# apache/arrow-rs

Measured on NVIDIA H100. Metric: Mrows/sec filter+take+add on 1e9-row Int64/Float64; % HBM roofline, higher is better.
Workload: dtype i64 (filter/take/sum) + f64 (add)

## Files before the change

arrow-rs_b200/csrc/bitmap.cu:

```cuda
#include "bitmap.cuh"

__global__ void __launch_bounds__(256) k_bitmap_and(const uint8_t *__restrict__ a, int64_t aoff,
                                                    const uint8_t *__restrict__ b, int64_t boff,
                                                    int64_t len, uint64_t *__restrict__ out,
                                                    unsigned long long *__restrict__ res) {
  int64_t words = (len + 63) >> 6;
  int64_t stride = (int64_t)gridDim.x * blockDim.x;
  unsigned cnt = 0;
  for (int64_t w = (int64_t)blockIdx.x * blockDim.x + threadIdx.x; w < words; w += stride) {
    uint64_t x = ld_bits64(a, aoff + (w << 6), aoff + len);
    if (b) x &= ld_bits64(b, boff + (w << 6), boff + len);
    if (out) out[w] = x;
    cnt += __popcll(x);
  }
  if (res) {
    cnt = warp_sum(cnt);
    if ((threadIdx.x & 31) == 0 && cnt) atomicAdd(res + RES_COUNT, (unsigned long long)cnt);
  }
}

acu_status acu_bitmap_and_launch(acu_ctx *ctx, const uint8_t *a, int64_t aoff, const uint8_t *b,
                                 int64_t boff, int64_t len, uint64_t *out, bool count, unsigned long long *res) {
  if (len <= 0) return ACU_OK;
  int64_t words = (len + 63) >> 6;
  ACU_LAUNCH(ctx, k_bitmap_and, acu_grid(ctx, (words + 255) / 256, 8), 256, 0, a, aoff, b, boff, len, out,
             count ? (res ? res : ctx->d_res) : nullptr);
  return ACU_OK;
}

int64_t acu_resolve_null_count(acu_ctx *ctx, const acu_array *a, acu_status *st) {
  *st = ACU_OK;
  if (!a->validity) return 0;
  if (a->null_count >= 0) return a->null_count;
  int64_t len = a->is_scalar ? 1 : a->len;
  if (len == 0) return 0;
  if (ctx->async_on) {
    *st = acu_fail(ctx, ACU_ERR_INVALID_ARGUMENT, -1, 0, 0, 0,
                   "null_count = -1 needs a device count (a synchronisation): pass the cached null_count inside an async section");
    return 0;
  }
  if ((*st = acu_res_reset(ctx)) != ACU_OK) return 0;
  if ((*st = acu_bitmap_and_launch(ctx, a->validity, a->validity_offset, nullptr, 0, len, nullptr, true)) != ACU_OK) return 0;
  if ((*st = acu_res_fetch(ctx)) != ACU_OK) return 0;
  return len - (int64_t)ctx->h_res[RES_COUNT];
}

extern "C" acu_status acu_bitmap_count(acu_ctx *ctx, const uint8_t *bits, int64_t offset,
                                       const uint8_t *validity, int64_t validity_offset, int64_t len,
                                       int64_t *out_count) {
  ACU_ENTER(ctx);
  *out_count = 0;
  if (len <= 0) return ACU_OK;
  ACU_TRY(acu_res_reset(ctx));
  ACU_TRY(acu_bitmap_and_launch(ctx, bits, offset, validity, validity_offset, len, nullptr, true));
  ACU_TRY(acu_res_fetch(ctx));
  *out_count = (int64_t)ctx->h_res[RES_COUNT];
  return ACU_OK;
}
```

arrow-rs_b200/csrc/elementwise.cu:

```cuda
#include <stdio.h>

#include <algorithm>
#include <limits>
#include <type_traits>

#include "bitmap.cuh"
#include "internal.cuh"

namespace {

template <class T, int EPL> struct alignas(EPL * sizeof(T) == 16 ? 16 : sizeof(T)) Pack { T v[EPL]; };

template <class T, int EPL>
__device__ __forceinline__ Pack<T, EPL> pack_load(const T *p) {
  Pack<T, EPL> r;
  if constexpr (EPL * sizeof(T) == 16) {
    uint4 x = ld_stream16(p);
    r = *reinterpret_cast<Pack<T, EPL> *>(&x);
  } else {
    static_assert(EPL == 1, "scalar path");
    r.v[0] = __ldg(p);
  }
  return r;
}
template <class T, int EPL>
__device__ __forceinline__ void pack_store(T *p, Pack<T, EPL> r) {
  if constexpr (EPL * sizeof(T) == 16) {
    st_stream16(p, *reinterpret_cast<uint4 *>(&r));
  } else {
    *p = r.v[0];
  }
}

__device__ __forceinline__ uint64_t ones_to(int64_t row, int64_t n) {
  int64_t k = n - row;
  return k >= 64 ? ~0ull : (k <= 0 ? 0ull : ((~0ull) >> (64 - k)));
}

enum { CLS_WRAP = 0, CLS_CHECKED = 1, CLS_DIVREM = 2, CLS_DECIMAL = 3 };
enum { OP_ADD = 0, OP_SUB = 1, OP_MUL = 2, OP_DIV = 3, OP_REM = 4, OP_NEG = 5 };

template <class T> struct is_fp { static constexpr bool value = std::is_floating_point<T>::value; };

__device__ __forceinline__ double fp_add(double a, double b) { return __dadd_rn(a, b); }
__device__ __forceinline__ double fp_sub(double a, double b) { return __dsub_rn(a, b); }
__device__ __forceinline__ double fp_mul(double a, double b) { return __dmul_rn(a, b); }
__device__ __forceinline__ double fp_div(double a, double b) { return __ddiv_rn(a, b); }
__device__ __forceinline__ double fp_rem(double a, double b) { return fmod(a, b); }
__device__ __forceinline__ float fp_add(float a, float b) { return __fadd_rn(a, b); }
__device__ __forceinline__ float fp_sub(float a, float b) { return __fsub_rn(a, b); }
__device__ __forceinline__ float fp_mul(float a, float b) { return __fmul_rn(a, b); }
__device__ __forceinline__ float fp_div(float a, float b) { return __fdiv_rn(a, b); }
__device__ __forceinline__ float fp_rem(float a, float b) { return fmodf(a, b); }

template <class T, int CLS>
__device__ __forceinline__ bool apply_op(int op, T l, T r, T &o) {
  if constexpr (is_fp<T>::value) {
    if constexpr (CLS == CLS_DIVREM) {
      o = (op == OP_DIV) ? fp_div(l, r) : fp_rem(l, r);
    } else {
      o = (op == OP_ADD) ? fp_add(l, r) : (op == OP_SUB) ? fp_sub(l, r) : (op == OP_MUL) ? fp_mul(l, r) : -r;
    }
    return false;
  } else {
    using U = typename std::make_unsigned<T>::type;
    constexpr bool SIGNED = std::is_signed<T>::value;
    if constexpr (CLS == CLS_WRAP) {
      U a = (U)l, b = (U)r;
      o = (T)((op == OP_ADD) ? (U)(a + b) : (op == OP_SUB) ? (U)(a - b) : (op == OP_MUL) ? (U)(a * b) : (U)((U)0 - b));
      return false;
    } else if constexpr (CLS == CLS_CHECKED) {
      if constexpr (sizeof(T) < 8) {
        using W = typename std::conditional<SIGNED, int64_t, uint64_t>::type;
        W a = (W)l, b = (W)r;
        W w = (op == OP_ADD) ? a + b : (op == OP_SUB) ? a - b : (op == OP_MUL) ? a * b : (W)0 - b;
        o = (T)w;
        if constexpr (SIGNED) return w < (W)std::numeric_limits<T>::min() || w > (W)std::numeric_limits<T>::max();
        else return (op == OP_SUB) ? (a < b) : (op == OP_NEG ? false : w > (W)std::numeric_limits<T>::max());
      } else if constexpr (SIGNED) {
        int64_t a = l, b = r;
        if (op == OP_NEG) { a = 0; }
        if (op == OP_ADD) {
          int64_t s = (int64_t)((uint64_t)a + (uint64_t)b);
          o = s;
          return ((a ^ s) & (b ^ s)) < 0;
        } else if (op == OP_MUL) {
          int64_t lo = (int64_t)((uint64_t)a * (uint64_t)b);
          int64_t hi = __mul64hi(a, b);
          o = lo;
          return hi != (lo >> 63);
        } else {
          int64_t s = (int64_t)((uint64_t)a - (uint64_t)b);
          o = s;
          return ((a ^ b) & (a ^ s)) < 0;
        }
      } else {
        uint64_t a = l, b = r;
        if (op == OP_ADD) { o = a + b; return o < a; }
        if (op == OP_MUL) { o = a * b; return __umul64hi(a, b) != 0; }
        if (op == OP_NEG) { o = (uint64_t)0 - b; return false; }
        o = a - b;
        return a < b;
      }
    } else {
      o = 0;
      if (r == 0) return true;
      if constexpr (SIGNED) {
        if (r == (T)-1) {
          if (op == OP_DIV) {
            if (l == std::numeric_limits<T>::min()) return true;
            o = (T)(-l);
          }
          return false;
        }
      }
      o = (op == OP_DIV) ? (T)(l / r) : (T)(l % r);
      return false;
    }
  }
}

template <class T> struct dec_unsigned;
template <> struct dec_unsigned<int32_t> { using type = uint32_t; };
template <> struct dec_unsigned<int64_t> { using type = uint64_t; };
template <> struct dec_unsigned<__int128> { using type = unsigned __int128; };
template <class T> __host__ __device__ __forceinline__ T dec_min() {
  return (T)((typename dec_unsigned<T>::type)1 << (8 * sizeof(T) - 1));
}

__host__ __device__ __forceinline__ uint64_t umul64hi(uint64_t a, uint64_t b) {
#ifdef __CUDA_ARCH__
  return __umul64hi(a, b);
#else
  return (uint64_t)(((unsigned __int128)a * b) >> 64);
#endif
}
__host__ __device__ __forceinline__ int64_t mul64hi(int64_t a, int64_t b) {
#ifdef __CUDA_ARCH__
  return __mul64hi(a, b);
#else
  return (int64_t)(((__int128)a * b) >> 64);
#endif
}

template <class T> __host__ __device__ __forceinline__ bool add_ovf(T a, T b, T &o) {
  using U = typename dec_unsigned<T>::type;
  const T s = (T)((U)a + (U)b);
  o = s;
  return ((a ^ s) & (b ^ s)) < 0;
}
template <class T> __host__ __device__ __forceinline__ bool sub_ovf(T a, T b, T &o) {
  using U = typename dec_unsigned<T>::type;
  const T s = (T)((U)a - (U)b);
  o = s;
  return ((a ^ b) & (a ^ s)) < 0;
}
__host__ __device__ __forceinline__ bool mul_ovf(int32_t a, int32_t b, int32_t &o) {
  const int64_t w = (int64_t)a * b;
  o = (int32_t)w;
  return w != (int64_t)o;
}
__host__ __device__ __forceinline__ bool mul_ovf(int64_t a, int64_t b, int64_t &o) {
  const int64_t lo = (int64_t)((uint64_t)a * (uint64_t)b);
  o = lo;
  return mul64hi(a, b) != (lo >> 63);
}
__host__ __device__ __forceinline__ bool mul_ovf(__int128 a, __int128 b, __int128 &o) {
  const int64_t a64 = (int64_t)a, b64 = (int64_t)b;
  if ((__int128)a64 == a && (__int128)b64 == b) {
    const uint64_t lo = (uint64_t)a64 * (uint64_t)b64;
    o = (__int128)(((unsigned __int128)(uint64_t)mul64hi(a64, b64) << 64) | lo);
    return false;
  }
  using U = unsigned __int128;
  const bool neg = (a < 0) != (b < 0);
  const U ua = a < 0 ? (U)0 - (U)a : (U)a, ub = b < 0 ? (U)0 - (U)b : (U)b;
  const uint64_t ah = (uint64_t)(ua >> 64), al = (uint64_t)ua, bh = (uint64_t)(ub >> 64), bl = (uint64_t)ub;
  if (ah && bh) return true;
  const uint64_t x = ah ? ah : bh, y = ah ? bl : al;
  if (umul64hi(x, y)) return true;
  const uint64_t cross = x * y;
  const uint64_t hi = umul64hi(al, bl) + cross;
  if (hi < cross) return true;
  const U m = ((U)hi << 64) | (U)(al * bl);
  if (m > ((U)1 << 127) - (neg ? 0 : 1)) return true;
  o = neg ? (__int128)((U)0 - m) : (__int128)m;
  return false;
}
template <class T> __host__ __device__ __forceinline__ bool divrem_ovf(bool is_div, T l, T r, T &o) {
  o = T();
  if (r == T()) return true;
  if (r == (T)-1) {
    if (l == dec_min<T>()) return true;
    if (is_div) o = (T)(T() - l);
    return false;
  }
  if constexpr (sizeof(T) == 16) {
    const int64_t l64 = (int64_t)l, r64 = (int64_t)r;
    if ((__int128)l64 == l && (__int128)r64 == r) {
      o = is_div ? l64 / r64 : l64 % r64;
      return false;
    }
  }
  o = is_div ? (T)(l / r) : (T)(l % r);
  return false;
}
template <class T> __host__ __device__ __forceinline__ bool dec_apply(int op, T l, T r, T l_mul, T r_mul, T &o) {
  o = T();
  if (op == OP_NEG) return sub_ovf<T>(T(), r, o);
  if (op == OP_MUL) return mul_ovf(l, r, o);
  if (l_mul != (T)1 && mul_ovf(l, l_mul, l)) return true;
  if (r_mul != (T)1 && mul_ovf(r, r_mul, r)) return true;
  if (op == OP_ADD) return add_ovf<T>(l, r, o);
  if (op == OP_SUB) return sub_ovf<T>(l, r, o);
  return divrem_ovf<T>(op == OP_DIV, l, r, o);
}

template <class T>
struct ArithParams {
  const T *a, *b;
  T *out;
  int64_t n;
  const uint8_t *av, *bv;
  int64_t aoff, boff;
  uint64_t *out_valid;
  unsigned long long *res;
  int op;
  int a_scalar, b_scalar;
  int zero_nulls;
  T l_mul, r_mul;
};

template <class T, int CLS>
__device__ __forceinline__ bool row_op(const ArithParams<T> &p, T l, T r, T &o) {
  if constexpr (CLS == CLS_DECIMAL) return dec_apply<T>(p.op, l, r, p.l_mul, p.r_mul, o);
  else return apply_op<T, CLS>(p.op, l, r, o);
}

template <class T, int CLS, int EPL>
__global__ void __launch_bounds__(256, (CLS == CLS_WRAP ? 4 : (CLS == CLS_DECIMAL && sizeof(T) == 16) ? 2 : 3))
    k_arith(const ArithParams<T> p) {
  constexpr bool WIDE = CLS == CLS_DECIMAL && sizeof(T) == 16;
  constexpr int R = (32 * EPL > 64) ? 32 * EPL : 64;
  constexpr int LPS = R / (32 * EPL);
  constexpr int U = (LPS >= 2 && !WIDE) ? 2 : 4;
  constexpr int GROUP = U * R;
  constexpr int SG = 2048;
  constexpr int GPS = SG / GROUP;
  constexpr bool fallible = (CLS != CLS_WRAP) && !is_fp<T>::value;
  const int lane = threadIdx.x & 31;
  const int64_t warp = ((int64_t)blockIdx.x * blockDim.x + threadIdx.x) >> 5;
  const int64_t nwarps = ((int64_t)gridDim.x * blockDim.x) >> 5;
  const int64_t n = p.n;
  const int64_t sgroups = n / SG;
  const bool has_valid = p.out_valid != nullptr;
  T sa = T(), sb = T();
  if (p.a_scalar) sa = ldg_elem(p.a);
  if (p.b_scalar) sb = ldg_elem(p.b);
  unsigned valid_cnt = 0;
  unsigned long long err = ~0ull;

  for (int64_t sg = warp; sg < sgroups; sg += nwarps) {
    const int64_t sbase = sg * SG;
    uint64_t vw = ~0ull;
    if (has_valid) {
      const int64_t row = sbase + lane * 64;
      if (p.av) vw &= ld_bits64(p.av, p.aoff + row, p.aoff + n);
      if (p.bv) vw &= ld_bits64(p.bv, p.boff + row, p.boff + n);
      p.out_valid[row >> 6] = vw;
      valid_cnt += __popcll(vw);
    }
#pragma unroll 1
    for (int gi = 0; gi < GPS; ++gi) {
      const int64_t base = sbase + gi * GROUP;
      const T *__restrict__ pa = p.a + base + lane * EPL;
      const T *__restrict__ pb = p.b + base + lane * EPL;
      Pack<T, EPL> va[U * LPS], vb[U * LPS];
#pragma unroll
      for (int k = 0; k < U * LPS; ++k) {
        if (!p.a_scalar) va[k] = pack_load<T, EPL>(pa + k * 32 * EPL);
        if (!p.b_scalar) vb[k] = pack_load<T, EPL>(pb + k * 32 * EPL);
      }
      T *__restrict__ po = p.out + base + lane * EPL;
#pragma unroll
      for (int k = 0; k < U * LPS; ++k) {
        uint32_t bits = ~0u;
        if (fallible && p.zero_nulls) {
          const int pos = gi * GROUP + k * 32 * EPL + lane * EPL;
          const uint64_t w = __shfl_sync(ACU_FULL_MASK, vw, pos >> 6);
          bits = (uint32_t)(w >> (pos & 63));
        }
        Pack<T, EPL> o;
#pragma unroll
        for (int e = 0; e < EPL; ++e) {
          const T l = p.a_scalar ? sa : va[k].v[e];
          const T r = p.b_scalar ? sb : vb[k].v[e];
          T x;
          const bool bad = row_op<T, CLS>(p, l, r, x);
          if (fallible) {
            if (!((bits >> e) & 1u)) x = T();
            else if (bad) {
              const unsigned long long i = (unsigned long long)(base + k * 32 * EPL + lane * EPL + e);
              err = i < err ? i : err;
            }
          }
          o.v[e] = x;
        }
        pack_store<T, EPL>(po + k * 32 * EPL, o);
      }
    }
  }

  if (warp == 0) {
    for (int64_t row = sgroups * SG; row < n; row += 64) {
      uint64_t vw = ones_to(row, n);
      if (has_valid) {
        if (p.av) vw &= ld_bits64(p.av, p.aoff + row, p.aoff + n);
        if (p.bv) vw &= ld_bits64(p.bv, p.boff + row, p.boff + n);
        if (lane == 0) { p.out_valid[row >> 6] = vw; valid_cnt += __popcll(vw); }
      }
#pragma unroll
      for (int h = 0; h < 2; ++h) {
        const int64_t i = row + h * 32 + lane;
        if (i >= n) continue;
        const T l = p.a_scalar ? sa : ldg_elem(p.a + i);
        const T r = p.b_scalar ? sb : ldg_elem(p.b + i);
        T x;
        const bool bad = row_op<T, CLS>(p, l, r, x);
        if (fallible) {
          const bool live = !p.zero_nulls || ((vw >> (h * 32 + lane)) & 1ull);
          if (!live) x = T();
          else if (bad) err = (unsigned long long)i < err ? (unsigned long long)i : err;
        }
        p.out[i] = x;
      }
    }
  }
  if (has_valid) {
    valid_cnt = warp_sum(valid_cnt);
    if (lane == 0 && valid_cnt) atomicAdd(p.res + RES_COUNT, (unsigned long long)valid_cnt);
  }
  if (fallible && err != ~0ull) atomicMin(p.res + RES_ERR_INDEX, err);
}

template <class T, int CLS>
acu_status launch_arith(acu_ctx *ctx, const ArithParams<T> &p) {
  constexpr int EPLV = 16 / sizeof(T);
  bool aligned = ((uintptr_t)p.out % 16 == 0) && (p.a_scalar || (uintptr_t)p.a % 16 == 0) &&
                 (p.b_scalar || (uintptr_t)p.b % 16 == 0);
  if (aligned) {
    int64_t blocks = (p.n / 2048 + 1 + 7) / 8;
    ACU_LAUNCH_TIMED(ctx, ACU_K_ARITH, (k_arith<T, CLS, EPLV>), acu_wave_grid(ctx, k_arith<T, CLS, EPLV>, 256, 0, blocks), 256, 0, p);
  } else {
    int64_t blocks = (p.n / 2048 + 1 + 7) / 8;
    ACU_LAUNCH_TIMED(ctx, ACU_K_ARITH, (k_arith<T, CLS, 1>), acu_wave_grid(ctx, k_arith<T, CLS, 1>, 256, 0, blocks), 256, 0, p);
  }
  return ACU_OK;
}

const char *op_symbol(acu_arith_op op) {
  switch (op) {
    case ACU_ADD_WRAPPING: case ACU_ADD: return "+";
    case ACU_SUB_WRAPPING: case ACU_SUB: return "-";
    case ACU_MUL_WRAPPING: case ACU_MUL: return "*";
    case ACU_DIV: return "/";
    default: return "%";
  }
}

void fmt_i128(char *buf, size_t n, __int128 v) {
  char tmp[48];
  int k = 0;
  unsigned __int128 m = v < 0 ? (unsigned __int128)0 - (unsigned __int128)v : (unsigned __int128)v;
  do { tmp[k++] = (char)('0' + (int)(m % 10)); m /= 10; } while (m);
  size_t j = 0;
  if (v < 0 && j + 1 < n) buf[j++] = '-';
  while (k && j + 1 < n) buf[j++] = tmp[--k];
  buf[j] = 0;
}
template <class T> void fmt_native(char *buf, size_t n, T v) {
  if constexpr (sizeof(T) == 16) fmt_i128(buf, n, v);
  else if constexpr (std::is_floating_point<T>::value) snprintf(buf, n, "%.17g", (double)v);
  else if constexpr (std::is_signed<T>::value) snprintf(buf, n, "%lld", (long long)v);
  else snprintf(buf, n, "%llu", (unsigned long long)v);
}
template <class T> uint64_t bits_of(T v) { uint64_t b = 0; memcpy(&b, &v, sizeof(T) < 8 ? sizeof(T) : 8); return b; }

template <class T> struct DecArgs {
  T l_mul, r_mul;
  int max_precision, max_scale;
  uint8_t precision;
  int8_t scale;
};

acu_status decimal_validate(acu_ctx *ctx, int max_precision, int max_scale, int precision, int scale) {
  if (precision == 0)
    return acu_fail(ctx, ACU_ERR_INVALID_ARGUMENT, -1, 0, 0, 0, "precision cannot be 0, has to be between [1, %d]", max_precision);
  if (precision > max_precision)
    return acu_fail(ctx, ACU_ERR_INVALID_ARGUMENT, -1, 0, 0, 0, "precision %d is greater than max %d", precision, max_precision);
  if (scale > max_scale)
    return acu_fail(ctx, ACU_ERR_INVALID_ARGUMENT, -1, 0, 0, 0, "scale %d is greater than max %d", scale, max_scale);
  if (scale > 0 && scale > precision)
    return acu_fail(ctx, ACU_ERR_INVALID_ARGUMENT, -1, 0, 0, 0, "scale %d is greater than precision %d", scale, precision);
  return ACU_OK;
}

template <class T>
acu_status arith_error(acu_ctx *ctx, acu_arith_op op, bool is_neg, const acu_array *a, const acu_array *b, int64_t idx,
                       const DecArgs<T> *dec = nullptr) {
  T l = T(), r = T();
  if (a) ACU_CUDA(ctx, cudaMemcpyAsync(&l, static_cast<const T *>(a->values) + (a->is_scalar ? 0 : idx), sizeof(T), cudaMemcpyDeviceToHost, ctx->stream));
  ACU_CUDA(ctx, cudaMemcpyAsync(&r, static_cast<const T *>(b->values) + (b->is_scalar ? 0 : idx), sizeof(T), cudaMemcpyDeviceToHost, ctx->stream));
  ACU_CUDA(ctx, cudaStreamSynchronize(ctx->stream));
  const uint64_t lb = bits_of(l), rb = bits_of(r);
  T x = l, y = r;
  const char *sym = op_symbol(op);
  bool rescale_failed = false;
  if constexpr (std::is_same<T, int32_t>::value || std::is_same<T, int64_t>::value || sizeof(T) == 16) {
    if (dec && !is_neg && op != ACU_MUL && op != ACU_MUL_WRAPPING) {
      T t;
      if (dec->l_mul != (T)1 && mul_ovf(l, dec->l_mul, t)) {
        y = dec->l_mul, rescale_failed = true;
      } else {
        if (dec->l_mul != (T)1) x = t;
        if (dec->r_mul != (T)1 && mul_ovf(r, dec->r_mul, t)) x = r, y = dec->r_mul, rescale_failed = true;
        else if (dec->r_mul != (T)1) y = t;
      }
      if (rescale_failed) sym = "*";
    }
  }
  if ((op == ACU_DIV || op == ACU_REM) && !is_neg && !rescale_failed && y == T())
    return acu_fail(ctx, ACU_ERR_DIVIDE_BY_ZERO, idx, lb, rb, 0, "Divide by zero error");
  char ls[48], rs[48];
  fmt_native(ls, sizeof ls, x);
  fmt_native(rs, sizeof rs, y);
  if (is_neg)
    return acu_fail(ctx, ACU_ERR_ARITHMETIC_OVERFLOW, idx, rb, 0, 0, "Overflow happened on: - %s", rs);
  return acu_fail(ctx, ACU_ERR_ARITHMETIC_OVERFLOW, idx, lb, rb, 0, "Overflow happened on: %s %s %s", ls, sym, rs);
}

template <class T, bool DEC = false>
acu_status arith_typed(acu_ctx *ctx, acu_arith_op op, const acu_array *a, const acu_array *b, acu_array_out *out,
                       const DecArgs<T> *dec = nullptr) {
  const bool checked = DEC || (!is_fp<T>::value && (op == ACU_ADD || op == ACU_SUB || op == ACU_MUL || op == ACU_DIV || op == ACU_REM));
  DecArgs<T> dv{};
  if constexpr (DEC) dv = *dec;
  auto validate = [ctx, dv]() -> acu_status {
    return DEC ? decimal_validate(ctx, dv.max_precision, dv.max_scale, dv.precision, dv.scale) : ACU_OK;
  };
  const bool a_s = a->is_scalar != 0, b_s = b->is_scalar != 0;
  acu_status st;
  ArithParams<T> p{};
  p.a = static_cast<const T *>(a->values);
  p.b = static_cast<const T *>(b->values);
  p.out = static_cast<T *>(out->values);
  p.res = ctx->d_res;
  p.a_scalar = a_s && !b_s;
  p.b_scalar = b_s && !a_s;
  switch (op) {
    case ACU_ADD_WRAPPING: case ACU_ADD: p.op = OP_ADD; break;
    case ACU_SUB_WRAPPING: case ACU_SUB: p.op = OP_SUB; break;
    case ACU_MUL_WRAPPING: case ACU_MUL: p.op = OP_MUL; break;
    case ACU_DIV: p.op = OP_DIV; break;
    default: p.op = OP_REM; break;
  }
  p.l_mul = DEC ? dv.l_mul : T();
  p.r_mul = DEC ? dv.r_mul : T();
  out->has_validity = 0;
  out->null_count = 0;
  int64_t len;
  if (a_s != b_s) {
    const acu_array *s = a_s ? a : b, *arr = a_s ? b : a;
    len = arr->len;
    int64_t snc = acu_resolve_null_count(ctx, s, &st);
    ACU_TRY(st);
    if (snc != 0) {
      ACU_TRY(acu_new_null(ctx, len, (size_t)len * sizeof(T), out));
      return validate();
    }
    out->len = len;
    if (len == 0) { out->has_validity = arr->validity != nullptr; return validate(); }
    if (arr->validity) {
      (a_s ? p.bv : p.av) = arr->validity;
      (a_s ? p.boff : p.aoff) = arr->validity_offset;
      p.out_valid = reinterpret_cast<uint64_t *>(out->validity);
      p.zero_nulls = checked;
    }
  } else {
    if (a->len != b->len)
      return acu_fail(ctx, ACU_ERR_COMPUTE, -1, 0, 0, 0,
                      checked ? "Cannot perform a binary operation on arrays of different length"
                              : "Cannot perform binary operation on arrays of different length");
    len = a->len;
    out->len = len;
    if (len == 0) return validate();
    int64_t an = acu_resolve_null_count(ctx, a, &st);
    ACU_TRY(st);
    int64_t bn = acu_resolve_null_count(ctx, b, &st);
    ACU_TRY(st);
    if (a->validity && b->validity && (an > 0 || bn > 0)) {
      p.av = a->validity; p.aoff = a->validity_offset;
      p.bv = b->validity; p.boff = b->validity_offset;
    } else if (a->validity && !b->validity && an > 0) {
      p.av = a->validity; p.aoff = a->validity_offset;
    } else if (b->validity && !a->validity && bn > 0) {
      p.bv = b->validity; p.boff = b->validity_offset;
    }
    if (p.av || p.bv) {
      p.out_valid = reinterpret_cast<uint64_t *>(out->validity);
      p.zero_nulls = checked;
    }
  }
  p.n = len;
  const int blk = acu_call_begin(ctx, &st);
  ACU_TRY(st);
  p.res = acu_dres(ctx, blk);
  if constexpr (DEC) {
    ACU_TRY((launch_arith<T, CLS_DECIMAL>(ctx, p)));
  } else if (is_fp<T>::value) {
    if (op == ACU_DIV || op == ACU_REM) ACU_TRY((launch_arith<T, CLS_DIVREM>(ctx, p)));
    else ACU_TRY((launch_arith<T, CLS_WRAP>(ctx, p)));
  } else if (op == ACU_DIV || op == ACU_REM) {
    ACU_TRY((launch_arith<T, CLS_DIVREM>(ctx, p)));
  } else if (checked) {
    ACU_TRY((launch_arith<T, CLS_CHECKED>(ctx, p)));
  } else {
    ACU_TRY((launch_arith<T, CLS_WRAP>(ctx, p)));
  }
  const acu_array ca = *a, cb = *b;
  const bool has_valid = p.out_valid != nullptr;
  return acu_call_end(ctx, blk, [ctx, op, checked, ca, cb, has_valid, len, out, dv, validate](const unsigned long long *h) -> acu_status {
    if (checked && h[RES_ERR_INDEX] != ~0ull) return arith_error<T>(ctx, op, false, &ca, &cb, (int64_t)h[RES_ERR_INDEX], DEC ? &dv : nullptr);
    if (has_valid) {
      out->has_validity = 1;
      out->null_count = len - (int64_t)h[RES_COUNT];
    }
    return validate();
  });
}

template <class T>
acu_status neg_typed(acu_ctx *ctx, int32_t checked_in, const acu_array *a, acu_array_out *out) {
  constexpr bool DEC = sizeof(T) == 16;
  const bool checked = DEC || (checked_in && !is_fp<T>::value);
  int64_t len = a->len;
  out->len = len;
  out->has_validity = a->validity != nullptr;
  out->null_count = 0;
  if (len == 0) return ACU_OK;
  ArithParams<T> p{};
  p.a = static_cast<const T *>(a->values);
  p.b = static_cast<const T *>(a->values);
  p.out = static_cast<T *>(out->values);
  p.res = ctx->d_res;
  p.a_scalar = 1;
  p.op = OP_NEG;
  p.n = len;
  if (a->validity) {
    p.bv = a->validity;
    p.boff = a->validity_offset;
    p.out_valid = reinterpret_cast<uint64_t *>(out->validity);
    p.zero_nulls = checked;
  }
  if constexpr (DEC) {
    acu_status st;
    const int blk = acu_call_begin(ctx, &st);
    ACU_TRY(st);
    p.res = acu_dres(ctx, blk);
    p.l_mul = p.r_mul = 1;
    ACU_TRY((launch_arith<T, CLS_DECIMAL>(ctx, p)));
    const acu_array ca = *a;
    const bool has_valid = p.out_valid != nullptr;
    return acu_call_end(ctx, blk, [ctx, ca, has_valid, len, out](const unsigned long long *h) -> acu_status {
      if (h[RES_ERR_INDEX] != ~0ull) return arith_error<T>(ctx, ACU_SUB, true, nullptr, &ca, (int64_t)h[RES_ERR_INDEX]);
      if (has_valid) out->null_count = len - (int64_t)h[RES_COUNT];
      return ACU_OK;
    });
  } else {
    ACU_TRY(acu_res_reset(ctx));
    if (checked) ACU_TRY((launch_arith<T, CLS_CHECKED>(ctx, p)));
    else ACU_TRY((launch_arith<T, CLS_WRAP>(ctx, p)));
    ACU_TRY(acu_res_fetch(ctx));
    if (checked && ctx->h_res[RES_ERR_INDEX] != ~0ull)
      return arith_error<T>(ctx, ACU_SUB, true, nullptr, a, (int64_t)ctx->h_res[RES_ERR_INDEX]);
    if (p.out_valid) out->null_count = len - (int64_t)ctx->h_res[RES_COUNT];
    return ACU_OK;
  }
}

template <class T>
struct CmpParams {
  const T *a, *b;
  int64_t n;
  const uint8_t *av, *bv;
  int64_t aoff, boff;
  int a_scalar, b_scalar;
  int a_null_scalar, b_null_scalar;
  int neg, fold;
  uint64_t *out_bits, *out_valid;
  unsigned long long *res;
  int fuse;
  uint32_t *tile_count;
};

template <class T> __device__ __forceinline__ bool pred_eq(T l, T r) {
  if constexpr (sizeof(T) == 8 && is_fp<T>::value) return __double_as_longlong(l) == __double_as_longlong(r);
  else if constexpr (is_fp<T>::value) return __float_as_int(l) == __float_as_int(r);
  else return l == r;
}
template <class T> __device__ __forceinline__ bool pred_lt(T l, T r) {
  if constexpr (is_fp<T>::value) return total_key(l) < total_key(r);
  else return l < r;
}

template <int EPL>
__device__ __forceinline__ void pack_lane_bits(uint32_t bits, int load, uint32_t &lo, uint32_t &hi) {
  const int lane = threadIdx.x & 31;
  bits <<= (lane * EPL) & 31;
  const int my_half = (lane * EPL) >> 5;
#pragma unroll
  for (int hh = 0; hh < EPL; ++hh) {
    const uint32_t half = __reduce_or_sync(ACU_FULL_MASK, my_half == hh ? bits : 0u);
    const int h = load * EPL + hh;
    if (lane == (h >> 1)) { if (h & 1) hi = half; else lo = half; }
  }
}

template <class T, bool LT, int EPL>
__global__ void __launch_bounds__(256, 4) k_cmp(const CmpParams<T> p) {
  constexpr int RPL = 32 * EPL;
  constexpr int LOADS = 2048 / RPL;
  constexpr int U = LOADS < 4 ? LOADS : 4;
  const int lane = threadIdx.x & 31;
  const int64_t warp = ((int64_t)blockIdx.x * blockDim.x + threadIdx.x) >> 5;
  const int64_t nwarps = ((int64_t)gridDim.x * blockDim.x) >> 5;
  const int64_t n = p.n;
  const int64_t sgroups = n >> 11;
  T sa = T(), sb = T();
  if (p.a_scalar) sa = ldg_elem(p.a);
  if (p.b_scalar) sb = ldg_elem(p.b);
  unsigned valid_cnt = 0;
  for (int64_t sg = warp; sg < sgroups; sg += nwarps) {
    const int64_t sbase = sg << 11;
    uint64_t lw = ~0ull, rw = ~0ull;
    if (p.a_null_scalar) lw = 0;
    if (p.b_null_scalar) rw = 0;
    const int64_t wrow = sbase + lane * 64;
    if (p.av) lw &= ld_bits64(p.av, p.aoff + wrow, p.aoff + n);
    if (p.bv) rw &= ld_bits64(p.bv, p.boff + wrow, p.boff + n);
    uint32_t my_lo = 0, my_hi = 0;
#pragma unroll 1
    for (int l0 = 0; l0 < LOADS; l0 += U) {
      Pack<T, EPL> va[U], vb[U];
#pragma unroll
      for (int u = 0; u < U; ++u) {
        const int64_t i0 = sbase + (int64_t)(l0 + u) * RPL + lane * EPL;
        if (!p.a_scalar) va[u] = pack_load<T, EPL>(p.a + i0);
        if (!p.b_scalar) vb[u] = pack_load<T, EPL>(p.b + i0);
      }
#pragma unroll
      for (int u = 0; u < U; ++u) {
        uint32_t x = 0;
#pragma unroll
        for (int e = 0; e < EPL; ++e) {
          const T l = p.a_scalar ? sa : va[u].v[e];
          const T r = p.b_scalar ? sb : vb[u].v[e];
          x |= (uint32_t)(LT ? pred_lt(l, r) : pred_eq(l, r)) << e;
        }
        pack_lane_bits<EPL>(x, l0 + u, my_lo, my_hi);
      }
    }
    uint64_t v = (uint64_t)my_lo | ((uint64_t)my_hi << 32);
    if (p.neg) v = ~v;
    if (p.fold == FOLD_DISTINCT) v = (lw ^ rw) | (lw & rw & v);
    else if (p.fold == FOLD_NOT_DISTINCT) v = ~(lw | rw) | (lw & rw & v);
    if (p.fuse) {
      if (p.fold == FOLD_NONE) v &= lw & rw;
      unsigned c = __popcll(v);
#pragma unroll
      for (int o = 8; o > 0; o >>= 1) c += __shfl_xor_sync(ACU_FULL_MASK, c, o);
      if ((lane & 15) == 0) p.tile_count[(sbase >> 10) + (lane >> 4)] = c;
    }
    p.out_bits[(sbase >> 6) + lane] = v;
    if (p.out_valid) {
      p.out_valid[(sbase >> 6) + lane] = lw & rw;
      valid_cnt += __popcll(lw & rw);
    }
  }

  if (warp == 0) {
    unsigned tile_cnt = 0;
    for (int64_t row = sgroups << 11; row < n; row += 64) {
      uint64_t v = 0;
#pragma unroll
      for (int h = 0; h < 2; ++h) {
        const int64_t i = row + h * 32 + lane;
        const T l = (!p.a_scalar && i < n) ? ldg_elem(p.a + i) : sa;
        const T r = (!p.b_scalar && i < n) ? ldg_elem(p.b + i) : sb;
        v |= (uint64_t)__ballot_sync(ACU_FULL_MASK, LT ? pred_lt(l, r) : pred_eq(l, r)) << (h * 32);
      }
      if (p.neg) v = ~v;
      if (lane == 0) {
        const uint64_t m = ones_to(row, n);
        v &= m;
        uint64_t lw = p.a_null_scalar ? 0ull : m, rw = p.b_null_scalar ? 0ull : m;
        if (p.av) lw &= ld_bits64(p.av, p.aoff + row, p.aoff + n);
        if (p.bv) rw &= ld_bits64(p.bv, p.boff + row, p.boff + n);
        if (p.fold == FOLD_DISTINCT) v = (lw ^ rw) | (lw & rw & v);
        else if (p.fold == FOLD_NOT_DISTINCT) v = (~(lw | rw) & m) | (lw & rw & v);
        else if (p.fuse) v &= lw & rw;
        p.out_bits[row >> 6] = v;
        if (p.out_valid) {
          p.out_valid[row >> 6] = lw & rw;
          valid_cnt += __popcll(lw & rw);
        }
        if (p.fuse) {
          tile_cnt += __popcll(v);
          if (row + 64 >= n || ((row + 64) & 1023) == 0) { p.tile_count[row >> 10] = tile_cnt; tile_cnt = 0; }
        }
      }
    }
  }
  if (p.out_valid) {
    valid_cnt = warp_sum(valid_cnt);
    if (lane == 0 && valid_cnt) atomicAdd(p.res + RES_COUNT, (unsigned long long)valid_cnt);
  }
}

template <class T, int EPL>
acu_status launch_cmp(acu_ctx *ctx, bool lt, const CmpParams<T> &p) {
  const int64_t blocks = (p.n / 2048 + 1 + 7) / 8;
  if (lt) ACU_LAUNCH_TIMED(ctx, ACU_K_CMP, (k_cmp<T, true, EPL>), acu_wave_grid(ctx, k_cmp<T, true, EPL>, 256, 0, blocks), 256, 0, p);
  else ACU_LAUNCH_TIMED(ctx, ACU_K_CMP, (k_cmp<T, false, EPL>), acu_wave_grid(ctx, k_cmp<T, false, EPL>, 256, 0, blocks), 256, 0, p);
  return ACU_OK;
}

struct CmpFuse {
  uint64_t *mask;
  int64_t n_words_padded;
  uint32_t *tile_count;
  int64_t n_tiles;
};

template <class T>
acu_status cmp_typed(acu_ctx *ctx, acu_cmp_op op, const acu_array *l, const acu_array *r, acu_array_out *out, const CmpFuse *fuse = nullptr) {
  acu_array_out scratch_out{};
  if (fuse) out = &scratch_out;
  acu_cmp_decision d;
  ACU_TRY(acu_cmp_decide(ctx, op, l, r, out, &d));
  const int64_t len = d.len;
  if (len == 0) return ACU_OK;
  if (fuse) {
    const int64_t used = (len + 63) / 64;
    if (fuse->n_words_padded > used)
      ACU_CUDA(ctx, cudaMemsetAsync(fuse->mask + used, 0, (size_t)(fuse->n_words_padded - used) * 8, ctx->stream));
  }
  if (d.all_null) {
    if (fuse) {
      ACU_CUDA(ctx, cudaMemsetAsync(fuse->mask, 0, (size_t)fuse->n_words_padded * 8, ctx->stream));
      ACU_CUDA(ctx, cudaMemsetAsync(fuse->tile_count, 0, (size_t)fuse->n_tiles * 4, ctx->stream));
      return ACU_OK;
    }
    return acu_new_null(ctx, len, acu_bitmap_bytes(len), out);
  }
  CmpParams<T> p{};
  p.a = static_cast<const T *>((d.swap ? r : l)->values);
  p.b = static_cast<const T *>((d.swap ? l : r)->values);
  p.n = len;
  p.av = d.av; p.aoff = d.aoff;
  p.bv = d.bv; p.boff = d.boff;
  p.a_scalar = d.a_scalar; p.a_null_scalar = d.a_null_scalar;
  p.b_scalar = d.b_scalar; p.b_null_scalar = d.b_null_scalar;
  p.neg = d.neg;
  p.fold = d.fold;
  p.out_bits = fuse ? fuse->mask : static_cast<uint64_t *>(out->values);
  if (d.has_validity && !fuse) p.out_valid = reinterpret_cast<uint64_t *>(out->validity);
  p.res = ctx->d_res;
  if (fuse) { p.fuse = 1; p.tile_count = fuse->tile_count; }
  int blk = 0;
  if (!fuse) {
    acu_status st;
    blk = acu_call_begin(ctx, &st);
    ACU_TRY(st);
    p.res = acu_dres(ctx, blk);
  }
  const bool aligned = (p.a_scalar || (uintptr_t)p.a % 16 == 0) && (p.b_scalar || (uintptr_t)p.b % 16 == 0);
  if (aligned) ACU_TRY((launch_cmp<T, 16 / sizeof(T)>(ctx, d.lt, p)));
  else ACU_TRY((launch_cmp<T, 1>(ctx, d.lt, p)));
  if (fuse) return ACU_OK;
  return acu_call_end(ctx, blk, [d, out](const unsigned long long *h) -> acu_status {
    acu_cmp_finalize(d, h, out);
    return ACU_OK;
  });
}

template <class I, class O>
__device__ __forceinline__ bool num_cast(I v, O &o) {
  if constexpr (is_fp<O>::value) {
    o = (O)v;
    return true;
  } else if constexpr (is_fp<I>::value) {
    if (v != v) return false;
    constexpr bool OS = std::is_signed<O>::value;
    if constexpr (sizeof(I) > sizeof(O)) {
      const I lo = OS ? (I)std::numeric_limits<O>::min() - (I)1 : (I)-1;
      const I hi = (I)std::numeric_limits<O>::max() + (I)1;
      if (!(v > lo && v < hi)) return false;
    } else {
      const I hi = (I)std::numeric_limits<O>::max();
      if constexpr (OS) { if (!(v >= (I)std::numeric_limits<O>::min() && v < hi)) return false; }
      else { if (!(v > (I)-1 && v < hi)) return false; }
    }
    o = (O)v;
    return true;
  } else {
    constexpr bool IS = std::is_signed<I>::value, OS = std::is_signed<O>::value;
    if constexpr (IS == OS) {
      if (v < std::numeric_limits<O>::min() || v > std::numeric_limits<O>::max()) return false;
    } else if constexpr (IS) {
      if (v < 0) return false;
      if ((typename std::make_unsigned<I>::type)v > std::numeric_limits<O>::max()) return false;
    } else {
      if (v > (typename std::make_unsigned<O>::type)std::numeric_limits<O>::max()) return false;
    }
    o = (O)v;
    return true;
  }
}

template <class I, class O> struct cast_infallible {
  static constexpr bool value = is_fp<O>::value ||
      (!is_fp<I>::value && ((std::is_signed<I>::value == std::is_signed<O>::value && sizeof(O) >= sizeof(I)) ||
                            (!std::is_signed<I>::value && std::is_signed<O>::value && sizeof(O) > sizeof(I))));
};
template <class O, int EPL> struct alignas((sizeof(O) * EPL >= 16) ? 16 : sizeof(O) * EPL) OutPack { O v[EPL]; };

template <class I, class O, int EPL>
__global__ void __launch_bounds__(256, 4) k_cast(const I *__restrict__ in, O *__restrict__ out, const int64_t n,
                                                 const uint8_t *__restrict__ iv, const int64_t ioff, uint64_t *__restrict__ out_valid,
                                                 const int safe, unsigned long long *__restrict__ res) {
  constexpr bool fallible = !cast_infallible<I, O>::value;
  constexpr int RPL = 32 * EPL;
  constexpr int LOADS = 2048 / RPL;
  constexpr int U = LOADS < 4 ? LOADS : 4;
  const int lane = threadIdx.x & 31;
  const int64_t warp = ((int64_t)blockIdx.x * blockDim.x + threadIdx.x) >> 5;
  const int64_t nwarps = ((int64_t)gridDim.x * blockDim.x) >> 5;
  const int64_t sgroups = n >> 11;
  unsigned valid_cnt = 0;
  unsigned long long err = ~0ull;
  for (int64_t sg = warp; sg < sgroups; sg += nwarps) {
    const int64_t sbase = sg << 11;
    uint64_t vw = ~0ull;
    if (iv) vw = ld_bits64(iv, ioff + sbase + lane * 64, ioff + n);
    uint32_t bad_lo = 0, bad_hi = 0;
#pragma unroll 1
    for (int l0 = 0; l0 < LOADS; l0 += U) {
      Pack<I, EPL> v[U];
#pragma unroll
      for (int u = 0; u < U; ++u) v[u] = pack_load<I, EPL>(in + sbase + (int64_t)(l0 + u) * RPL + lane * EPL);
#pragma unroll
      for (int u = 0; u < U; ++u) {
        const int pos = (l0 + u) * RPL + lane * EPL;
        const uint64_t w = __shfl_sync(ACU_FULL_MASK, vw, pos >> 6);
        const uint32_t bits = (uint32_t)(w >> (pos & 63));
        OutPack<O, EPL> o;
        uint32_t bad = 0;
#pragma unroll
        for (int e = 0; e < EPL; ++e) {
          O x = O();
          if (((bits >> e) & 1u) && !num_cast<I, O>(v[u].v[e], x)) bad |= 1u << e;
          o.v[e] = x;
        }
        *reinterpret_cast<OutPack<O, EPL> *>(out + sbase + pos) = o;
        if (fallible && __any_sync(ACU_FULL_MASK, bad)) pack_lane_bits<EPL>(bad, l0 + u, bad_lo, bad_hi);
      }
    }
    const uint64_t bad = (uint64_t)bad_lo | ((uint64_t)bad_hi << 32);
    if (fallible && bad) {
      if (safe) vw &= ~bad;
      else err = min(err, (unsigned long long)(sbase + lane * 64 + __ffsll((long long)bad) - 1));
    }
    if (out_valid) { out_valid[(sbase >> 6) + lane] = vw; valid_cnt += __popcll(vw); }
  }

  if (warp == 0) {
    for (int64_t row = sgroups << 11; row < n; row += 64) {
      uint64_t vw = ones_to(row, n);
      if (iv) vw &= ld_bits64(iv, ioff + row, ioff + n);
      uint64_t bad = 0;
#pragma unroll
      for (int h = 0; h < 2; ++h) {
        const int64_t i = row + h * 32 + lane;
        O x = O();
        const bool b = ((vw >> (h * 32 + lane)) & 1ull) && !num_cast<I, O>(__ldg(in + i), x);
        if (i < n) out[i] = x;
        if constexpr (fallible) bad |= (uint64_t)__ballot_sync(ACU_FULL_MASK, b) << (h * 32);
      }
      if (fallible && bad) {
        if (safe) vw &= ~bad;
        else err = min(err, (unsigned long long)(row + __ffsll((long long)bad) - 1));
      }
      if (out_valid && lane == 0) { out_valid[row >> 6] = vw; valid_cnt += __popcll(vw); }
    }
  }
  if (out_valid) {
    valid_cnt = warp_sum(valid_cnt);
    if (lane == 0 && valid_cnt) atomicAdd(res + RES_COUNT, (unsigned long long)valid_cnt);
  }
  if (fallible && err != ~0ull) atomicMin(res + RES_ERR_INDEX, err);
}

template <class I, class O>
acu_status cast_typed(acu_ctx *ctx, acu_dtype to, int32_t safe, const acu_array *a, acu_array_out *out) {
  const int64_t len = a->len;
  out->len = len;
  out->null_count = 0;
  out->has_validity = safe ? 1 : (a->validity != nullptr);
  if (len == 0) return ACU_OK;
  uint64_t *ov = out->has_validity ? reinterpret_cast<uint64_t *>(out->validity) : nullptr;
  ACU_TRY(acu_res_reset(ctx));
  const I *in = static_cast<const I *>(a->values);
  O *o = static_cast<O *>(out->values);
  constexpr int EPLV = sizeof(I) == 8 ? 1 : 16 / sizeof(I);
  const int64_t blocks = (len / 2048 + 1 + 7) / 8;
  if ((uintptr_t)in % 16 == 0 && (uintptr_t)o % 16 == 0)
    ACU_LAUNCH_TIMED(ctx, ACU_K_CAST, (k_cast<I, O, EPLV>), acu_wave_grid(ctx, k_cast<I, O, EPLV>, 256, 0, blocks), 256, 0,
                     in, o, len, a->validity, a->validity_offset, ov, safe, ctx->d_res);
  else
    ACU_LAUNCH_TIMED(ctx, ACU_K_CAST, (k_cast<I, O, 1>), acu_wave_grid(ctx, k_cast<I, O, 1>, 256, 0, blocks), 256, 0,
                     in, o, len, a->validity, a->validity_offset, ov, safe, ctx->d_res);
  ACU_TRY(acu_res_fetch(ctx));
  if (!safe && ctx->h_res[RES_ERR_INDEX] != ~0ull) {
    const int64_t idx = (int64_t)ctx->h_res[RES_ERR_INDEX];
    I v;
    ACU_CUDA(ctx, cudaMemcpyAsync(&v, static_cast<const I *>(a->values) + idx, sizeof(I), cudaMemcpyDeviceToHost, ctx->stream));
    ACU_CUDA(ctx, cudaStreamSynchronize(ctx->stream));
    char s[40];
    fmt_native(s, sizeof s, v);
    return acu_fail(ctx, ACU_ERR_CAST, idx, bits_of(v), 0, 0, "Can't cast value %s to type %s", s, acu_dtype_name(to));
  }
  if (ov) out->null_count = len - (int64_t)ctx->h_res[RES_COUNT];
  return ACU_OK;
}

template <class I>
acu_status cast_from(acu_ctx *ctx, acu_dtype to, int32_t safe, const acu_array *a, acu_array_out *out) {
  switch (to) {
    case ACU_I8: return cast_typed<I, int8_t>(ctx, to, safe, a, out);
    case ACU_I16: return cast_typed<I, int16_t>(ctx, to, safe, a, out);
    case ACU_I32: return cast_typed<I, int32_t>(ctx, to, safe, a, out);
    case ACU_I64: return cast_typed<I, int64_t>(ctx, to, safe, a, out);
    case ACU_U8: return cast_typed<I, uint8_t>(ctx, to, safe, a, out);
    case ACU_U16: return cast_typed<I, uint16_t>(ctx, to, safe, a, out);
    case ACU_U32: return cast_typed<I, uint32_t>(ctx, to, safe, a, out);
    case ACU_U64: return cast_typed<I, uint64_t>(ctx, to, safe, a, out);
    case ACU_F32: return cast_typed<I, float>(ctx, to, safe, a, out);
    case ACU_F64: return cast_typed<I, double>(ctx, to, safe, a, out);
  }
  return acu_fail(ctx, ACU_ERR_NOT_YET_IMPLEMENTED, -1, 0, 0, 0, "cast to dtype %d", (int)to);
}

acu_status i128_aligned(acu_ctx *ctx, const void *x, const void *y) {
  if (((uintptr_t)x | (uintptr_t)y) % 16 != 0)
    return acu_fail(ctx, ACU_ERR_INVALID_ARGUMENT, -1, 0, 0, 0, "Int128 values must be 16-byte aligned");
  return ACU_OK;
}

int8_t i8_wrap(int v) { return (int8_t)(uint8_t)(v & 0xff); }
int8_t i8_sat(int v) { return (int8_t)(v < -128 ? -128 : v > 127 ? 127 : v); }
uint8_t u8_sat(int v) { return (uint8_t)(v > 255 ? 255 : v); }
uint8_t u8_of(int8_t v) { return (uint8_t)v; }
uint32_t u32_of(int8_t v) { return (uint32_t)(int32_t)v; }

template <class T> bool pow10_checked(uint32_t exp, T *out) {
  T v = 1;
  for (uint32_t i = 0; i < exp; ++i)
    if (mul_ovf(v, (T)10, v)) return false;
  *out = v;
  return true;
}
template <class T> T pow10_wrapping(uint32_t exp) {
  using U = typename dec_unsigned<T>::type;
  if (exp >= 8 * sizeof(T)) return T();
  U v = 1;
  for (uint32_t i = 0; i < exp; ++i) v *= 10;
  return (T)v;
}

const char *decimal_name(int width) { return width == 4 ? "Decimal32" : width == 8 ? "Decimal64" : "Decimal128"; }

template <class T>
acu_status decimal_typed(acu_ctx *ctx, acu_arith_op op, const acu_decimal_type &lt, const acu_array *a, const acu_decimal_type &rt,
                         const acu_array *b, acu_decimal_type *out_type, acu_array_out *out) {
  constexpr int MP = sizeof(T) == 4 ? 9 : sizeof(T) == 8 ? 18 : 38;
  const int p1 = lt.precision, p2 = rt.precision, s1 = lt.scale, s2 = rt.scale;
  DecArgs<T> d{};
  d.l_mul = d.r_mul = 1;
  d.max_precision = d.max_scale = MP;
  uint32_t le = 0, re = 0;
  bool pow_l = false, pow_r = false;
  switch (op) {
    case ACU_ADD: case ACU_ADD_WRAPPING: case ACU_SUB: case ACU_SUB_WRAPPING: case ACU_REM: {
      const int8_t rs = (int8_t)(s1 > s2 ? s1 : s2);
      const int8_t d1 = i8_wrap(p1 - s1), d2 = i8_wrap(p2 - s2);
      if (op == ACU_REM) {
        d.precision = (uint8_t)std::min<int>(u8_of(i8_sat(rs + std::min(d1, d2))), MP);
        d.l_mul = pow10_wrapping<T>(u32_of(i8_wrap(rs - s1)));
        d.r_mul = pow10_wrapping<T>(u32_of(i8_wrap(rs - s2)));
      } else {
        d.precision = (uint8_t)std::min<int>(u8_sat(u8_of(i8_sat(rs + std::max(d1, d2))) + 1), MP);
        le = u32_of(i8_wrap(rs - s1));
        re = u32_of(i8_wrap(rs - s2));
        pow_l = pow_r = true;
      }
      d.scale = rs;
      break;
    }
    case ACU_MUL: case ACU_MUL_WRAPPING: {
      d.precision = (uint8_t)std::min<int>(u8_sat(p1 + p2 + 1), MP);
      d.scale = i8_sat(s1 + s2);
      if (d.scale > MP)
        return acu_fail(ctx, ACU_ERR_INVALID_ARGUMENT, -1, 0, 0, 0, "Output scale of %s(%d, %d) * %s(%d, %d) would exceed max scale of %d",
                        decimal_name(lt.byte_width), p1, s1, decimal_name(rt.byte_width), p2, s2, MP);
      break;
    }
    case ACU_DIV: {
      const int8_t rs = (int8_t)std::min<int>(i8_sat(s1 + 4), MP);
      const int8_t mul_pow = i8_wrap(i8_wrap(rs - s1) + s2);
      d.precision = (uint8_t)std::min<int>(u8_of(i8_sat(mul_pow + p1)), MP);
      d.scale = rs;
      if (mul_pow > 0) { le = u32_of(mul_pow); pow_l = true; }
      else if (mul_pow < 0) { re = u32_of(i8_wrap(-mul_pow)); pow_r = true; }
      break;
    }
    default:
      return acu_fail(ctx, ACU_ERR_INVALID_ARGUMENT, -1, 0, 0, 0, "Invalid arithmetic operation: op %d", (int)op);
  }
  if (pow_l && !pow10_checked<T>(le, &d.l_mul))
    return acu_fail(ctx, ACU_ERR_ARITHMETIC_OVERFLOW, -1, 0, 0, 0, "Overflow happened on: 10 ^ %u", le);
  if (pow_r && !pow10_checked<T>(re, &d.r_mul))
    return acu_fail(ctx, ACU_ERR_ARITHMETIC_OVERFLOW, -1, 0, 0, 0, "Overflow happened on: 10 ^ %u", re);
  out_type->byte_width = lt.byte_width;
  out_type->precision = d.precision;
  out_type->scale = d.scale;
  out_type->reserved[0] = out_type->reserved[1] = 0;
  return arith_typed<T, true>(ctx, op, a, b, out, &d);
}

}

#define ACU_DISPATCH(dt, F, ...)                         \
  switch (dt) {                                          \
    case ACU_I8: return F<int8_t>(__VA_ARGS__);          \
    case ACU_I16: return F<int16_t>(__VA_ARGS__);        \
    case ACU_I32: return F<int32_t>(__VA_ARGS__);        \
    case ACU_I64: return F<int64_t>(__VA_ARGS__);        \
    case ACU_U8: return F<uint8_t>(__VA_ARGS__);         \
    case ACU_U16: return F<uint16_t>(__VA_ARGS__);       \
    case ACU_U32: return F<uint32_t>(__VA_ARGS__);       \
    case ACU_U64: return F<uint64_t>(__VA_ARGS__);       \
    case ACU_F32: return F<float>(__VA_ARGS__);          \
    case ACU_F64: return F<double>(__VA_ARGS__);         \
  }

extern "C" acu_status acu_arith(acu_ctx *ctx, acu_dtype dtype, acu_arith_op op, const acu_array *a,
                                const acu_array *b, acu_array_out *out) {
  ACU_ENTER(ctx);
  ACU_DISPATCH(dtype, arith_typed, ctx, op, a, b, out)
  return acu_fail(ctx, ACU_ERR_INVALID_ARGUMENT, -1, 0, 0, 0, "Invalid arithmetic operation: dtype %d", (int)dtype);
}

extern "C" acu_status acu_neg(acu_ctx *ctx, acu_dtype dtype, int32_t checked, const acu_array *a, acu_array_out *out) {
  ACU_ENTER(ctx);
  if (checked && (dtype == ACU_U8 || dtype == ACU_U16 || dtype == ACU_U32 || dtype == ACU_U64))
    return acu_fail(ctx, ACU_ERR_INVALID_ARGUMENT, -1, 0, 0, 0, "Invalid arithmetic operation: !%s", acu_dtype_name(dtype));
  ACU_DISPATCH(dtype, neg_typed, ctx, checked, a, out)
  if (dtype == ACU_I128) {
    ACU_TRY(i128_aligned(ctx, a->values, out->values));
    return neg_typed<__int128>(ctx, 1, a, out);
  }
  return acu_fail(ctx, ACU_ERR_INVALID_ARGUMENT, -1, 0, 0, 0, "Invalid arithmetic operation: dtype %d", (int)dtype);
}

extern "C" acu_status acu_cmp(acu_ctx *ctx, acu_dtype dtype, acu_cmp_op op, const acu_array *a,
                              const acu_array *b, acu_array_out *out) {
  ACU_ENTER(ctx);
  ACU_DISPATCH(dtype, cmp_typed, ctx, op, a, b, out)
  if (dtype == ACU_I128) {
    ACU_TRY(i128_aligned(ctx, a->values, b->values));
    return cmp_typed<__int128>(ctx, op, a, b, out);
  }
  return acu_fail(ctx, ACU_ERR_INVALID_ARGUMENT, -1, 0, 0, 0, "Invalid comparison operation: dtype %d", (int)dtype);
}

acu_status acu_cmp_len(acu_ctx *ctx, const acu_array *l, const acu_array *r, int64_t *len) {
  const bool ls = l->is_scalar != 0, rs = r->is_scalar != 0;
  if (l->len != r->len && !ls && !rs)
    return acu_fail(ctx, ACU_ERR_INVALID_ARGUMENT, -1, 0, 0, 0,
                    "Cannot compare arrays of different lengths, got %lld vs %lld", (long long)l->len, (long long)r->len);
  *len = ls ? r->len : l->len;
  return ACU_OK;
}

acu_status acu_cmp_decide(acu_ctx *ctx, acu_cmp_op op, const acu_array *l, const acu_array *r, acu_array_out *out,
                          acu_cmp_decision *d) {
  *d = acu_cmp_decision{};
  ACU_TRY(acu_cmp_len(ctx, l, r, &d->len));
  out->len = d->len;
  out->has_validity = 0;
  out->null_count = 0;
  if (d->len == 0) return ACU_OK;
  acu_status st;
  const int64_t lnc = acu_resolve_null_count(ctx, l, &st);
  ACU_TRY(st);
  const int64_t rnc = acu_resolve_null_count(ctx, r, &st);
  ACU_TRY(st);
  const bool ls = l->is_scalar != 0, rs = r->is_scalar != 0;
  const bool ln = lnc > 0, rn = rnc > 0;
  const bool fold = op == ACU_DISTINCT || op == ACU_NOT_DISTINCT;
  d->all_null = !fold && ((ls && ln) || (rs && rn)) && !(ls && rs);
  if (d->all_null) return ACU_OK;
  d->swap = op == ACU_GT || op == ACU_LT_EQ;
  const acu_array *x = d->swap ? r : l, *y = d->swap ? l : r;
  const bool xs = d->swap ? rs : ls, ys = d->swap ? ls : rs;
  const bool xn = d->swap ? rn : ln, yn = d->swap ? ln : rn;
  d->lt = !(op == ACU_EQ || op == ACU_NEQ || fold);
  d->neg = op == ACU_NEQ || op == ACU_DISTINCT || op == ACU_LT_EQ || op == ACU_GT_EQ;
  d->fold = op == ACU_DISTINCT ? FOLD_DISTINCT : op == ACU_NOT_DISTINCT ? FOLD_NOT_DISTINCT : FOLD_NONE;
  d->a_scalar = xs && !ys;
  d->b_scalar = ys && !xs;
  if (xn) { if (d->a_scalar) d->a_null_scalar = 1; else { d->av = x->validity; d->aoff = x->validity_offset; } }
  if (yn) { if (d->b_scalar) d->b_null_scalar = 1; else { d->bv = y->validity; d->boff = y->validity_offset; } }
  d->has_validity = !fold && (xn || yn);
  return ACU_OK;
}

void acu_cmp_finalize(const acu_cmp_decision &d, const unsigned long long *hres, acu_array_out *out) {
  if (!d.has_validity) return;
  out->has_validity = 1;
  out->null_count = d.len - (int64_t)hres[RES_COUNT];
}

acu_status acu_new_null(acu_ctx *ctx, int64_t len, size_t value_bytes, acu_array_out *out) {
  if (value_bytes) ACU_CUDA(ctx, cudaMemsetAsync(out->values, 0, value_bytes, ctx->stream));
  if (len) ACU_CUDA(ctx, cudaMemsetAsync(out->validity, 0, acu_bitmap_bytes(len), ctx->stream));
  ACU_CUDA(ctx, cudaStreamSynchronize(ctx->stream));
  out->len = len;
  out->has_validity = 1;
  out->null_count = len;
  return ACU_OK;
}

acu_status acu_cmp_into_plan(acu_ctx *ctx, acu_dtype dtype, acu_cmp_op op, const acu_array *a, const acu_array *b, uint64_t *mask,
                             int64_t n_words_padded, uint32_t *tile_count, int64_t n_tiles) {
  CmpFuse f{mask, n_words_padded, tile_count, n_tiles};
  const CmpFuse *fuse = &f;
  acu_array_out *out = nullptr;
  ACU_DISPATCH(dtype, cmp_typed, ctx, op, a, b, out, fuse)
  if (dtype == ACU_I128) {
    ACU_TRY(i128_aligned(ctx, a->values, b->values));
    return cmp_typed<__int128>(ctx, op, a, b, out, fuse);
  }
  return acu_fail(ctx, ACU_ERR_INVALID_ARGUMENT, -1, 0, 0, 0, "Invalid comparison operation: dtype %d", (int)dtype);
}

extern "C" acu_status acu_cast_numeric(acu_ctx *ctx, acu_dtype from, acu_dtype to, int32_t safe,
                                       const acu_array *a, acu_array_out *out) {
  ACU_ENTER(ctx);
  ACU_DISPATCH(from, cast_from, ctx, to, safe, a, out)
  return acu_fail(ctx, ACU_ERR_NOT_YET_IMPLEMENTED, -1, 0, 0, 0, "cast from dtype %d", (int)from);
}

extern "C" acu_status acu_decimal_arith(acu_ctx *ctx, acu_arith_op op, const acu_decimal_type *lt, const acu_array *a,
                                        const acu_decimal_type *rt, const acu_array *b, acu_decimal_type *out_type,
                                        acu_array_out *out) {
  ACU_ENTER(ctx);
  const int w = lt->byte_width;
  if ((w != 4 && w != 8 && w != 16) || rt->byte_width != w)
    return acu_fail(ctx, ACU_ERR_INVALID_ARGUMENT, -1, 0, 0, 0, "Invalid decimal operation: byte widths %d and %d", (int)w, (int)rt->byte_width);
  const int mp = w == 4 ? 9 : w == 8 ? 18 : 38;
  ACU_TRY(decimal_validate(ctx, mp, mp, lt->precision, lt->scale));
  ACU_TRY(decimal_validate(ctx, mp, mp, rt->precision, rt->scale));
  if (w == 4) return decimal_typed<int32_t>(ctx, op, *lt, a, *rt, b, out_type, out);
  if (w == 8) return decimal_typed<int64_t>(ctx, op, *lt, a, *rt, b, out_type, out);
  ACU_TRY(i128_aligned(ctx, a->values, b->values));
  ACU_TRY(i128_aligned(ctx, out->values, nullptr));
  return decimal_typed<__int128>(ctx, op, *lt, a, *rt, b, out_type, out);
}
```

Baseline: 74460.

## Split arith validity AND into separate bitmap kernel with batched loads

When arithmetic produces an output validity bitmap and cannot fail on null-masked rows, the validity AND plus popcount now runs in a dedicated bitmap kernel, and the arith kernel runs without validity inputs. The bitmap kernel is restructured to issue K=4 raw word loads per thread before joining and shifting them, raising memory-level parallelism. This adds a second launch and a second pass over the bitmaps, in exchange for a leaner main arith loop.

```diff
diff --git a/arrow-rs_b200/csrc/bitmap.cu b/arrow-rs_b200/csrc/bitmap.cu
--- a/arrow-rs_b200/csrc/bitmap.cu
+++ b/arrow-rs_b200/csrc/bitmap.cu
@@ -1,17 +1,54 @@
 #include "bitmap.cuh"
+
+struct Bits64Raw {
+  uint64_t lo, hi;
+};
+__device__ __forceinline__ unsigned bits64_shift(const uint8_t *base, int64_t pos) {
+  return (unsigned)((((uintptr_t)base + (uintptr_t)(pos >> 3)) & 7) << 3) + (unsigned)(pos & 7);
+}
+__device__ __forceinline__ Bits64Raw ld_bits64_raw(const uint8_t *__restrict__ base, int64_t pos, int64_t end) {
+  const int64_t n = end - pos;
+  const unsigned shift = bits64_shift(base, pos);
+  const uint64_t *p = reinterpret_cast<const uint64_t *>(((uintptr_t)base + (uintptr_t)(pos >> 3)) & ~(uintptr_t)7);
+  Bits64Raw r;
+  r.lo = n > 0 ? __ldg(p) : 0ull;
+  r.hi = (n > 0 && shift != 0 && (int64_t)(64 - shift) < n) ? __ldg(p + 1) : 0ull;
+  return r;
+}
+__device__ __forceinline__ uint64_t bits64_join(const Bits64Raw &r, const uint8_t *base, int64_t pos, int64_t end) {
+  const int64_t n = end - pos;
+  if (n <= 0) return 0ull;
+  const unsigned shift = bits64_shift(base, pos);
+  uint64_t w = r.lo >> shift;
+  if (shift != 0) w |= r.hi << (64 - shift);
+  if (n < 64) w &= (~0ull) >> (64 - n);
+  return w;
+}
 
 __global__ void __launch_bounds__(256) k_bitmap_and(const uint8_t *__restrict__ a, int64_t aoff,
                                                     const uint8_t *__restrict__ b, int64_t boff,
                                                     int64_t len, uint64_t *__restrict__ out,
                                                     unsigned long long *__restrict__ res) {
+  constexpr int K = 4;
   int64_t words = (len + 63) >> 6;
   int64_t stride = (int64_t)gridDim.x * blockDim.x;
   unsigned cnt = 0;
-  for (int64_t w = (int64_t)blockIdx.x * blockDim.x + threadIdx.x; w < words; w += stride) {
-    uint64_t x = ld_bits64(a, aoff + (w << 6), aoff + len);
-    if (b) x &= ld_bits64(b, boff + (w << 6), boff + len);
-    if (out) out[w] = x;
-    cnt += __popcll(x);
+  for (int64_t w0 = (int64_t)blockIdx.x * blockDim.x + threadIdx.x; w0 < words; w0 += K * stride) {
+    Bits64Raw ra[K], rb[K];
+#pragma unroll
+    for (int k = 0; k < K; ++k) {
+      const int64_t w = w0 + k * stride;
+      ra[k] = ld_bits64_raw(a, aoff + (w << 6), aoff + len);
+      if (b) rb[k] = ld_bits64_raw(b, boff + (w << 6), boff + len);
+    }
+#pragma unroll
+    for (int k = 0; k < K; ++k) {
+      const int64_t w = w0 + k * stride;
+      uint64_t x = bits64_join(ra[k], a, aoff + (w << 6), aoff + len);
+      if (b) x &= bits64_join(rb[k], b, boff + (w << 6), boff + len);
+      if (out && w < words) out[w] = x;
+      cnt += __popcll(x);
+    }
   }
   if (res) {
     cnt = warp_sum(cnt);
diff --git a/arrow-rs_b200/csrc/elementwise.cu b/arrow-rs_b200/csrc/elementwise.cu
--- a/arrow-rs_b200/csrc/elementwise.cu
+++ b/arrow-rs_b200/csrc/elementwise.cu
@@ -344,7 +344,19 @@
 }
 
 template <class T, int CLS>
-acu_status launch_arith(acu_ctx *ctx, const ArithParams<T> &p) {
+acu_status launch_arith(acu_ctx *ctx, const ArithParams<T> &p_in) {
+  constexpr bool fallible = (CLS != CLS_WRAP) && !is_fp<T>::value;
+  ArithParams<T> p = p_in;
+  if (p.out_valid && !(fallible && p.zero_nulls)) {
+    const bool a_first = p.av != nullptr;
+    const int slot = acu_kstats_begin(ctx, ACU_K_ARITH);
+    const acu_status st = acu_bitmap_and_launch(ctx, a_first ? p.av : p.bv, a_first ? p.aoff : p.boff, a_first ? p.bv : nullptr,
+                                                a_first ? p.boff : 0, p.n, p.out_valid, true, p.res);
+    acu_kstats_end(ctx, slot);
+    ACU_TRY(st);
+    p.out_valid = nullptr;
+    p.av = p.bv = nullptr;
+  }
   constexpr int EPLV = 16 / sizeof(T);
   bool aligned = ((uintptr_t)p.out % 16 == 0) && (p.a_scalar || (uintptr_t)p.a % 16 == 0) &&
                  (p.b_scalar || (uintptr_t)p.b % 16 == 0);
```

New measurement: 74530 (median of 6 runs). Within noise of the previous version (+0.1%).
